# Healthcare-Robotics/assistive-gym

Hardware: AMD Instinct MI355X
Metric: env_steps_per_sec (higher is better)
Workload: dtype f32; 1 GPU; FeedingJaco-v1, 4096 lockstep envs per MI355X, random-policy rollout, 5 simulation steps per env step, 50 PGS sweeps; envs_per_gpu=4096, global_envs=4096, reset_pool=256, reset=pool, parallelism=env-sharded x1, obs_allgather=False

## Files before the change

### __graft_entry__.py

```python
import os
import subprocess
import sys

ROOT = os.path.dirname(os.path.abspath(__file__))
if ROOT not in sys.path:
    sys.path.insert(0, ROOT)


def build():
    from assistive_gym_amd.build import build as build_lib
    build_lib(force=True)
    build_lib(out=os.path.join(ROOT, 'assistive_gym_amd', 'lib', 'variants', 'lvs.so'), extra=('-DAGX_PGS_LV=3',), only=['FEEDING'])
    build_lib(out=os.path.join(ROOT, 'assistive_gym_amd', 'lib', 'variants', 'scan4.so'), extra=('-DAGX_GJK_SCAN_WIDE=0', '-DAGX_GJK_SCAN_ONE=0'), only=['FEEDING'])
    build_lib(out=os.path.join(ROOT, 'assistive_gym_amd', 'lib', 'variants', 'finishgjk.so'), extra=('-DAGX_FINISH_SPILL_GJK',), only=['FEEDING'])
    subprocess.check_call(['make', '-C', os.path.join(ROOT, 'oracle')], stdout=subprocess.DEVNULL)
    if os.path.isdir('/root/reference/assistive_gym/envs/assets'):
        from assistive_gym_amd.model import compiler
        compiler.main()
    import assistive_gym_amd
    from assistive_gym_amd import libagx
    L = libagx.load()
    missing = [e for e in libagx.EXPORTS if not hasattr(L, e)]
    assert not missing, missing


def smoke():
    import numpy as np
    sys.path.insert(0, os.path.join(ROOT, 'tests'))
    from assistive_gym_amd import libagx
    from assistive_gym_amd.blob import ModelBlob
    from assistive_gym_amd.vec_env import build_reset_pool
    from oracle_lib import Oracle
    libagx.check(libagx.load().agx_selftest(0), 'agx_selftest')
    n = 64
    for model in ('feeding_jaco', 'bed_bathing_sawyer'):
        blob = ModelBlob.load(model)
        states = build_reset_pool(blob, n, seed=1001)
        st = libagx.Stepper(blob, n)
        st.set_state(states)
        actions = np.random.RandomState(0).uniform(-1, 1, (n, blob.act_dim)).astype(np.float32)
        obs, rew, done, info = st.step_host(actions)
        o = Oracle(blob)
        worst = 0.0
        for i in range(8):
            o_obs, o_rew, _, o_info = o.step(states[i].copy(), actions[i])
            worst = max(worst, float(np.abs(obs[i] - o_obs).max()), abs(float(rew[i]) - o_rew))
        assert np.isfinite(obs).all() and np.isfinite(rew).all()
        assert worst < 1e-3, (model, worst)
        print('smoke ok: 64 %s envs stepped on the GPU (%s kernels), max |obs, reward| deviation from the oracle %.2e' % (model, st.variant(), worst))
        st.close()


if __name__ == '__main__':
    build()
    if len(sys.argv) > 1 and sys.argv[1] == 'smoke':
        smoke()
```

### assistive_gym_amd/csrc/agx_collide.h

```cpp
#pragma once

namespace agx {

struct Cand { v3 pa, pb, n; float dist, gap; };
constexpr float GJK_FAR_MARGIN = 1e-4f;

AGX_DEV void make_shape(const Ctx& c, int col, v3 shift, gjk_shape& s) {
  s.n = CLI(c, col, AGX_C_NVERT);
  s.v = c.bf + c.o_vert + 3 * CLI(c, col, AGX_C_VOFF);
  v3 p; body_xf(c, CLI(c, col, AGX_C_BODY), s.R, p);
  s.p = p - shift; s.box = false;
  s.c = mul(s.R, mk3(CLF(c, col, AGX_C_AABB_C), CLF(c, col, AGX_C_AABB_C + 1), CLF(c, col, AGX_C_AABB_C + 2))) + s.p;
}
AGX_DEV bool narrowphase(const Ctx& c, int ca, int cb, float limit, Cand& out, bool has) {
  const float* AB = c.lds + L_ARENA;
  gjk_shape sa, sb;
  sa.v = nullptr; sa.n = 0; sa.box = false; sa.c = mk3(0.f, 0.f, 0.f); sb.v = nullptr; sb.n = 0; sb.box = false; sb.c = sa.c;
  v3 shift = mk3(0.f, 0.f, 0.f);
  float ra = 0.f, rb = 0.f;
  bool ok = has;
  if (has) {
    shift = mk3(0.5f * (AB[ABS * ca] + AB[ABS * ca + 3]), 0.5f * (AB[ABS * ca + 1] + AB[ABS * ca + 4]), 0.5f * (AB[ABS * ca + 2] + AB[ABS * ca + 5]));
    make_shape(c, ca, shift, sa); make_shape(c, cb, shift, sb);
    if (CLI(c, cb, AGX_C_BODY) == AGX_BODY_WORLD && sb.n == 8 && (CLI(c, cb, AGX_C_TAG) == AGX_TAG_TABLE || CLI(c, cb, AGX_C_TAG) == AGX_TAG_PLANE)) {
      sb.box = true;
      float lo[3], hi[3];
      for (int k = 0; k < 3; k++) {
        lo[k] = fmaxf(AB[ABS * cb + k], AB[ABS * ca + k] - AGX_BOX_CLIP); hi[k] = fminf(AB[ABS * cb + 3 + k], AB[ABS * ca + 3 + k] + AGX_BOX_CLIP);
        if (hi[k] < lo[k]) ok = false;
      }
      sb.lo = mk3(lo[0], lo[1], lo[2]) - shift; sb.hi = mk3(hi[0], hi[1], hi[2]) - shift; sb.c = 0.5f * (sb.lo + sb.hi);
    }
    ra = CLF(c, ca, AGX_C_RADIUS); rb = CLF(c, cb, AGX_C_RADIUS);
  }
  float d; v3 pa, pb, n;
  const bool pen = gjk_distance(sa, sb, PRM(c, AGX_P_GJK_TOL), (int)PRM(c, AGX_P_GJK_MAXIT), limit + ra + rb + GJK_FAR_MARGIN, ok, d, pa, pb);
  if (!ok) return false;
  if (!pen) {
    if (d - ra - rb >= limit) return false;
    n = (1.0f / d) * (pa - pb);
  } else {
    float depth; gjk_penetration(sa, sb, c.bf + c.o_dirs, c.bi[AGX_H_NDIR], depth, n, pa, pb);
    d = -depth;
  }
  out.pa = pa - ra * n + shift; out.pb = pb + rb * n + shift; out.n = n; out.dist = d - ra - rb;
  return true;
}
AGX_DEV float pair_mu(const Ctx& c, int ca, int cb) {
  float plane_mu = c.lds[L_ST + c.s_env + AGX_E_PLANE_FRICTION];
  float mua = CLI(c, ca, AGX_C_TAG) == AGX_TAG_PLANE ? plane_mu : CLF(c, ca, AGX_C_FRICTION);
  float mub = CLI(c, cb, AGX_C_TAG) == AGX_TAG_PLANE ? plane_mu : CLF(c, cb, AGX_C_FRICTION);
  return mua * mub;
}
AGX_DEV void emit_contact(Ctx& c, int slot, int ca, int cb, const Cand& k) {
  float* o = c.gcon + CON_STRIDE * slot; int* oi = (int*)o;
  oi[C_CA] = ca; oi[C_CB] = cb; oi[C_BA] = CLI(c, ca, AGX_C_BODY); oi[C_BB] = CLI(c, cb, AGX_C_BODY);
  st3(o + C_PA, k.pa); st3(o + C_PB, k.pb); st3(o + C_N, k.n); o[C_DIST] = k.dist; o[C_MU] = pair_mu(c, ca, cb); o[C_LAM] = 0.f;
}
constexpr int CAND_STRIDE = 8;
constexpr int TW_WORDS = 6 * (MAX_DOF + MAX_FREE);
constexpr int WL_FIT = (ARENA_WORDS - ABS * MAX_COLL - TW_WORDS) / (1 + CAND_STRIDE);
constexpr int WL_MAX = WL_FIT < 200 ? WL_FIT : 200;
constexpr int A_WL = ABS * MAX_COLL;
constexpr int WL_KEY_MASK = ~((511 << 9) | (3 << 24));
constexpr int A_CAND = A_WL + WL_MAX;
constexpr int A_TW = A_CAND + WL_MAX * CAND_STRIDE;
static_assert(A_TW + TW_WORDS <= ARENA_WORDS, "collision workspace exceeds the arena");
static_assert(MAX_COLL <= 512, "collider indices are packed in 9 bits");
constexpr bool LIST_BYTES = MAX_COLL <= 256;
constexpr int LIST_TAIL = LIST_BYTES ? 8 : 16;
constexpr int WL_CAP = WL_MAX - LIST_TAIL;
template <bool B> struct ListIndex { typedef unsigned short type; };
template <> struct ListIndex<true> { typedef uint8_t type; };
typedef ListIndex<LIST_BYTES>::type list_t;
static_assert(WL_CAP >= 128, "a flush of at least two full passes");

AGX_DEV void emit_from_cand(Ctx& c, int slot, int idx) {
  const float* L = c.lds; const int pr = c.ldsi[L_ARENA + A_WL + idx]; const float* cd = L + L_ARENA + A_CAND + CAND_STRIDE * idx;
  Cand k; k.gap = cd[0]; k.pa = ld3(cd + 1); k.n = ld3(cd + 4); k.dist = cd[7]; k.pb = k.pa - k.dist * k.n;
  emit_contact(c, slot, pr & 511, (pr >> 9) & 511, k);
}
AGX_DEV bool face_box(const Ctx& c, int cb) {
  return CLI(c, cb, AGX_C_BODY) == AGX_BODY_WORLD && CLI(c, cb, AGX_C_NVERT) == 8 && (CLI(c, cb, AGX_C_TAG) == AGX_TAG_TABLE || CLI(c, cb, AGX_C_TAG) == AGX_TAG_PLANE);
}
AGX_DEV bool face_point(const Ctx& c, int ca, int cb, int e, v3 p0, Cand& out) {
  const float* AB = c.lds + L_ARENA;
  const int n = CLI(c, ca, AGX_C_NVERT);
  const float* V = c.bf + c.o_vert + 3 * CLI(c, ca, AGX_C_VOFF);
  m3 R; v3 p; body_xf(c, CLI(c, ca, AGX_C_BODY), R, p);
  const float x0 = AB[ABS * cb], y0 = AB[ABS * cb + 1], x1 = AB[ABS * cb + 3], y1 = AB[ABS * cb + 4], top = AB[ABS * cb + 5];
  float zmin = 3.0e38f;
  for (int v = 0; v < n; v++) { const v3 w = mul(R, mk3(V[3 * v], V[3 * v + 1], V[3 * v + 2])) + p; if (w.x >= x0 && w.x <= x1 && w.y >= y0 && w.y <= y1 && w.z < zmin) zmin = w.z; }
  float cx[1 + AGX_FACE_EXTRA], cy[1 + AGX_FACE_EXTRA];
  cx[0] = p0.x; cy[0] = p0.y;
#pragma unroll
  for (int q = 1; q <= AGX_FACE_EXTRA; q++) { cx[q] = 0.f; cy[q] = 0.f; }
  v3 pick = mk3(0.f, 0.f, 0.f);
  if (e == 0) {
    bool found = false;
    for (int v = 0; v < n && !found; v++) {
      const v3 w = mul(R, mk3(V[3 * v], V[3 * v + 1], V[3 * v + 2])) + p;
      if (w.x >= x0 && w.x <= x1 && w.y >= y0 && w.y <= y1 && w.z <= zmin + AGX_FACE_BAND) { pick = w; found = true; }
    }
    if (!found) return false;
  }
#pragma unroll
  for (int q = 1; q <= AGX_FACE_EXTRA; q++) {
    if (q > e) break;
    int bi = -1; float bd = AGX_FACE_SPREAD * AGX_FACE_SPREAD; v3 bw = mk3(0.f, 0.f, 0.f);
    for (int v = 0; v < n; v++) {
      const v3 w = mul(R, mk3(V[3 * v], V[3 * v + 1], V[3 * v + 2])) + p;
      if (!(w.x >= x0 && w.x <= x1 && w.y >= y0 && w.y <= y1) || w.z > zmin + AGX_FACE_BAND) continue;
      float dmin = 3.0e38f;
#pragma unroll
      for (int k = 0; k <= AGX_FACE_EXTRA; k++) if (k < q) { const float dx = w.x - cx[k], dy = w.y - cy[k]; dmin = fminf(dmin, dx * dx + dy * dy); }
      if (dmin > bd) { bd = dmin; bi = v; bw = w; }
    }
    if (bi < 0) return false;
    cx[q] = bw.x; cy[q] = bw.y; pick = bw;
  }
  const float ra = CLF(c, ca, AGX_C_RADIUS);
  out.n = mk3(0.f, 0.f, 1.f); out.pa = mk3(pick.x, pick.y, pick.z - ra); out.pb = mk3(pick.x, pick.y, top); out.dist = pick.z - ra - top;
  return true;
}
struct CollideState { int ncon, near_mask, overflow, maxc, nqpt; };
struct GroupRegs { int a0, a1, b0, b1, flags, keep; float alo[3], ahi[3], blo[3], bhi[3]; };
AGX_DEV float body_wmag(const Ctx& c, int code) {
  if (code >= 0 && code < AGX_BODY_ROBOT_BASE) return c.lds[L_WMAG + code];
  if (code >= AGX_BODY_FREE0 && code < AGX_BODY_HUMAN0) return c.lds[L_WMAG + MAX_DOF + (code - AGX_BODY_FREE0)];
  return 0.f;
}
AGX_DEV void body_twist(const Ctx& c, int code, v3& w, v3& v) {
  int slot = -1;
  if (code >= 0 && code < AGX_BODY_ROBOT_BASE) slot = code;
  else if (code >= AGX_BODY_FREE0 && code < AGX_BODY_HUMAN0) slot = MAX_DOF + (code - AGX_BODY_FREE0);
  if (slot < 0) { w = mk3(0.f, 0.f, 0.f); v = w; return; }
  const float* T = c.lds + L_ARENA + A_TW + 6 * slot;
  w = ld3(T); v = ld3(T + 3);
}
AGX_DEV float rel_travel(const Ctx& c, int a, int b) {
  const float* AB = c.lds + L_ARENA;
#ifdef AGX_NO_REL_TRAVEL
  return AB[ABS * a + 6] + AB[ABS * b + 6];
#endif
  v3 wa, va, wb, vb;
  body_twist(c, CLI(c, a, AGX_C_BODY), wa, va); body_twist(c, CLI(c, b, AGX_C_BODY), wb, vb);
  const bool sa = CLI(c, a, AGX_C_NVERT) == 1, sb = CLI(c, b, AGX_C_NVERT) == 1;
  const int e = (!sa && sb) ? b : a;
  const v3 lo = ld3(AB + ABS * e), hi = ld3(AB + ABS * e + 3);
  const v3 ce = 0.5f * (lo + hi), d = hi - lo;
  const v3 dw = wa - wb;
  const v3 u = (va - vb) + cross(dw, ce - ld3(c.lds + L_MISC + M_REF));
  const float rot = (sa || sb) ? 0.f : sqrtf(dot(dw, dw)) * 0.5f * sqrtf(dot(d, d));
  const float t = 1.001f * (sqrtf(dot(u, u)) + rot) * c.dt + 1e-6f;
  return fminf(t, AB[ABS * a + 6] + AB[ABS * b + 6]);
}
AGX_DEV bool sphere_box_apart(const Ctx& c, int x, int y, float reach) {
  const float* AB = c.lds + L_ARENA;
  const v3 cx = mk3(0.5f * (AB[ABS * x] + AB[ABS * x + 3]), 0.5f * (AB[ABS * x + 1] + AB[ABS * x + 4]), 0.5f * (AB[ABS * x + 2] + AB[ABS * x + 5]));
  const v3 hx = mk3(CLF(c, x, AGX_C_AABB_H), CLF(c, x, AGX_C_AABB_H + 1), CLF(c, x, AGX_C_AABB_H + 2));
  const float rx = sqrtf(dot(hx, hx)) + CLF(c, x, AGX_C_RADIUS);
  m3 R; v3 p; body_xf(c, CLI(c, y, AGX_C_BODY), R, p);
  const v3 pl = tmul(R, cx - p) - mk3(CLF(c, y, AGX_C_AABB_C), CLF(c, y, AGX_C_AABB_C + 1), CLF(c, y, AGX_C_AABB_C + 2));
  const float dx = fmaxf(fabsf(pl.x) - CLF(c, y, AGX_C_AABB_H), 0.f), dy = fmaxf(fabsf(pl.y) - CLF(c, y, AGX_C_AABB_H + 1), 0.f),
              dz = fmaxf(fabsf(pl.z) - CLF(c, y, AGX_C_AABB_H + 2), 0.f);
  const float lb = sqrtf(dx * dx + dy * dy + dz * dz) - rx - CLF(c, y, AGX_C_RADIUS);
  return lb > reach;
}

AGX_DEV void collide_flush(Ctx& c, int wn, CollideState& cs, float brk, float slack, const GroupRegs& G) {
  float* L = c.lds; int* WL = c.ldsi + L_ARENA + A_WL; float* CD = L + L_ARENA + A_CAND; const int lane = c.lane;
  const float* AB = L + L_ARENA;
  const int food0 = c.bi[AGX_H_FOOD0];
  if (wn == 0) return;
  wave_sync();
  long long ct0 = c.timing ? wave_clock() : 0;
  if (c.timing) { c.tm[13] += wn; c.tm[14] += (wn + 63) / 64; }
  bool any_manifold_query = false;
  for (int base = 0; base < wn; base += 64) {
    const int i = base + lane; const bool has = i < wn;
    Cand k; k.gap = 3.0e38f; bool near = false; int a = 0, g = 0;
    int b = 0, sub = 0;
    float lim = brk;
    if (has) {
      const int pr = WL[i]; a = pr & 511; b = (pr >> 9) & 511; g = (pr >> 18) & 63; sub = (pr >> 24) & 3;
      if (!(GRI(c, g, AGX_G_FLAGS) & (2 | 64))) lim = fminf(brk, slack + rel_travel(c, a, b) + 1e-5f);
    }
    k.n = mk3(0.f, 0.f, 0.f); k.pa = k.n; k.pb = k.n; k.dist = 0.f;
    bool hit = narrowphase(c, a, b, lim, k, has && sub == 0);
    if (has && sub == 0 && hit && k.n.z > 0.999f && face_box(c, b) && CLI(c, a, AGX_C_NVERT) >= 2) { Cand k0; k0.gap = k.gap; if (face_point(c, a, b, 0, k.pa, k0)) k = k0; }
    if (wave_any(has && sub > 0)) {
      if (has && sub == 0) { float* cd = CD + CAND_STRIDE * i; st3(cd + 1, k.pa); st3(cd + 4, k.n); }
      wave_sync();
      if (has && sub > 0) {
        const float* sd = CD + CAND_STRIDE * (i - sub);
        hit = sd[6] > 0.999f && face_point(c, a, b, sub, ld3(sd + 1), k) && k.dist < brk;
      }
    }
    if (has) {
      if (hit) {
        near = true;
        v3 vr = point_velocity(c, CLI(c, a, AGX_C_BODY), k.pa) - point_velocity(c, CLI(c, b, AGX_C_BODY), k.pb);
        float pg = k.dist + dot(vr, k.n) * c.dt;
        if (pg < ((GRI(c, g, AGX_G_FLAGS) & 64) ? brk : slack)) k.gap = pg;
      }
      float* cd = CD + CAND_STRIDE * i;
      cd[0] = k.gap; st3(cd + 1, k.pa); st3(cd + 4, k.n); cd[7] = k.dist;
    }
    if constexpr (TASK == AGX_TASK_FEEDING) {
      const bool mq = has && near && (GRI(c, g, AGX_G_FLAGS) & 2) && CLI(c, a, AGX_C_TAG) == AGX_TAG_FOOD;
      if (wave_any(mq)) { any_manifold_query = true; for (int f = 0; f < c.nfood; f++) if (wave_any(mq && CLI(c, a, AGX_C_BODY) - AGX_BODY_FREE0 - food0 == f)) cs.near_mask |= 1 << f; }
    }
    if constexpr (TASK != AGX_TASK_FEEDING) {
      const bool qp = has && near && (GRI(c, g, AGX_G_FLAGS) & 2) && CLI(c, a, AGX_C_TAG) == AGX_TAG_TOOL && (TKI(c, AGX_T_PAD_LINK) >> (CLI(c, a, AGX_C_LINK) + 1) & 1) &&
                      CLI(c, b, AGX_C_TAG) == AGX_TAG_HUMAN;
      const uint64_t qm = wave_ballot(qp);
      const int slot = cs.nqpt + wave_rank(qm);
      if (qp && slot < MAX_QPT) { float* o = c.gqpt + QPT_STRIDE * slot; st3(o, k.pb); ((int*)o)[3] = CLI(c, b, AGX_C_LINK); }
      cs.nqpt += popc64(qm);
    }
  }
  (void)any_manifold_query;
  wave_sync();
  if (c.timing) { long long t = wave_clock(); c.tm[11] += t - ct0; ct0 = t; }
  int* SEL = c.ldsi + L_ARENA + A_CAND + CAND_STRIDE * WL_CAP;
  const int ncon0 = cs.ncon;
  int cur = 0;
  while (cur < wn) {
    const int key = WL[cur] & WL_KEY_MASK;
    const int g = (key >> 18) & 63, keep = wave_bcast_i(G.keep, g);
    const int i0 = cur + lane, i1 = cur + 64 + lane;
    const bool s0 = i0 < wn && (WL[i0 < wn ? i0 : 0] & WL_KEY_MASK) == key, s1 = i1 < wn && (WL[i1 < wn ? i1 : 0] & WL_KEY_MASK) == key;
    const uint64_t b0 = wave_ballot(s0), b1 = wave_ballot(s1);
    const int len0 = (~b0) ? ffs64(~b0) : 64;
    const int len = len0 < 64 ? len0 : 64 + ((~b1) ? ffs64(~b1) : 64);
    const bool in0 = lane < len, in1 = 64 + lane < len;
    float g0 = in0 ? CD[CAND_STRIDE * i0] : 3.0e38f, g1 = in1 ? CD[CAND_STRIDE * i1] : 3.0e38f;
    if (keep == 0) {
      for (int pass = 0; pass < 2; pass++) {
        const bool has = (pass ? g1 : g0) < 1.0e38f;
        const uint64_t m = wave_ballot(has);
        int cnt = popc64(m); const int slot = cs.ncon + wave_rank(m);
        if (has && slot < cs.maxc) SEL[slot - ncon0] = pass ? i1 : i0;
        int room = cs.maxc - cs.ncon; if (room < 0) room = 0;
        if (cnt > room) { cs.overflow += cnt - room; cnt = room; }
        cs.ncon += cnt;
      }
    } else {
      for (int q = 0; q < keep; q++) {
        const float mg = wave_min(fminf(g0, g1));
        if (mg > 1.0e38f) break;
        const uint64_t m0 = wave_ballot(g0 == mg);
        int slot1 = 0, win;
        if (m0) win = ffs64(m0); else { win = ffs64(wave_ballot(g1 == mg)); slot1 = 1; }
        if (cs.ncon < cs.maxc) { if (lane == win) SEL[cs.ncon - ncon0] = slot1 ? i1 : i0; cs.ncon++; } else cs.overflow++;
        if (lane == win) { if (slot1) g1 = 3.0e38f; else g0 = 3.0e38f; }
      }
    }
    cur += len;
  }
  wave_sync();
  if (ncon0 + lane < cs.ncon) emit_from_cand(c, ncon0 + lane, SEL[lane]);
  wave_sync();
  if (c.timing) { long long t = wave_clock(); c.tm[12] += t - ct0; }
}

AGX_DEV int collide_sweep(Ctx& c, int g, int aa, int ab, int b0, int b1, int gflags, float mg, int wn, int rep, const GroupRegs& G) {
  const float* AB = c.lds + L_ARENA; int* WL = c.ldsi + L_ARENA + A_WL; const int lane = c.lane;
  const bool same = gflags & 1, no_adjacent = gflags & 4;
  float ulo[2][3], uhi[2][3];
  for (int q = 0; q < 3; q++) { ulo[0][q] = wave_bcast(G.blo[q], g); uhi[0][q] = wave_bcast(G.bhi[q], g); ulo[1][q] = wave_bcast(G.alo[q], g); uhi[1][q] = wave_bcast(G.ahi[q], g); }
  list_t* LIST = (list_t*)(c.ldsi + L_ARENA + A_CAND + CAND_STRIDE * WL_CAP);
  int nlive[2] = {0, 0};
  for (int side = 0; side < 2; side++) {
    const int r0 = side == 0 ? aa : b0, r1 = side == 0 ? ab : b1;
    for (int base = r0; base < r1; base += 64) {
      const int x = base + lane; bool ok = x < r1;
      if (ok) for (int q = 0; q < 3; q++) if (AB[ABS * x + q] > uhi[side][q] + mg || ulo[side][q] > AB[ABS * x + 3 + q] + mg) ok = false;
      const uint64_t m = wave_ballot(ok);
      if (ok) LIST[128 * side + nlive[side] + wave_rank(m)] = (list_t)x;
      nlive[side] += popc64(m);
    }
  }
  const int na_live = nlive[0], nb = nlive[1];
  wave_sync();
  const int npairs = na_live * nb * rep;
  for (int base = 0; base < npairs; base += 64) {
    const int p = base + lane; bool ok = p < npairs;
    const int pq = ok ? p / rep : 0, sub = ok ? p - pq * rep : 0;
    const int ai = pq / nb; const int a = LIST[ai], b = LIST[128 + pq - ai * nb];
    ok = ok && (!same || b > a) && (sub == 0 || (face_box(c, b) && CLI(c, a, AGX_C_NVERT) >= 2));
    if (ok && no_adjacent) {
      const int la = CLI(c, a, AGX_C_BODY), lb = CLI(c, b, AGX_C_BODY);
      if (la == lb) ok = false;
      else if (la >= 0 && la < AGX_BODY_ROBOT_BASE && lb >= 0 && lb < AGX_BODY_ROBOT_BASE && (RBI(c, la, AGX_R_PARENT) == lb || RBI(c, lb, AGX_R_PARENT) == la)) ok = false;
    }
    if (ok) for (int q = 0; q < 3; q++) if (AB[ABS * a + q] > AB[ABS * b + 3 + q] + mg || AB[ABS * b + q] > AB[ABS * a + 3 + q] + mg) ok = false;
    if (ok) { const float reach = mg + rel_travel(c, a, b) + 1e-5f; ok = !sphere_box_apart(c, a, b, reach) && (CLI(c, a, AGX_C_NVERT) == 1 || !sphere_box_apart(c, b, a, reach)); }
    const uint64_t m = wave_ballot(ok);
    const int slot = wn + wave_rank(m);
    if (ok && slot < WL_CAP) WL[slot] = a | (b << 9) | (g << 18) | (sub << 24);
    wn += popc64(m);
  }
  wave_sync();
  return wn;
}

AGX_DEV void collide(Ctx& c) {
  float* L = c.lds; float* AB = L + L_ARENA; const int lane = c.lane;
  const float brk = PRM(c, AGX_P_CONTACT_BREAK), slack = PRM(c, AGX_P_CONTACT_SLACK);
  CollideState cs; cs.ncon = 0; cs.near_mask = 0; cs.overflow = 0; cs.nqpt = 0;
  cs.maxc = (int)PRM(c, AGX_P_MAX_CONTACTS); if (cs.maxc > MAX_CON) cs.maxc = MAX_CON;
  long long ct0 = c.timing ? wave_clock() : 0, ct1;
#define AGX_CTICK(k) if (c.timing) { ct1 = wave_clock(); c.tm[k] += ct1 - ct0; ct0 = ct1; }
  if (lane < MAX_DOF + MAX_FREE) {
    v3 w = mk3(0, 0, 0), v = w;
    if (lane < MAX_DOF) { if (lane < c.ndof) for (int d = lane; d >= 0; d = RBI(c, d, AGX_R_PARENT)) { const float qd = L[L_VEL + d]; w = w + qd * ld3(L + L_S + 6 * d); v = v + qd * ld3(L + L_S + 6 * d + 3); } }
    else if (lane - MAX_DOF < c.nfree) {
      const int fb = lane - MAX_DOF, o = c.ndof + 6 * fb;
      w = ld3(L + L_VEL + o + 3);
      v = ld3(L + L_VEL + o) + cross(w, ld3(L + L_MISC + M_REF) - ld3(L + L_ST + c.s_free + 13 * fb));
    }
    L[L_WMAG + lane] = sqrtf(dot(w, w));
    st3(AB + A_TW + 6 * lane, w); st3(AB + A_TW + 6 * lane + 3, v);
  }
  wave_sync();
  for (int col = lane; col < c.ncoll; col += 64) {
    const int code = CLI(c, col, AGX_C_BODY);
    m3 R; v3 p; body_xf(c, code, R, p);
    v3 cl = mk3(CLF(c, col, AGX_C_AABB_C), CLF(c, col, AGX_C_AABB_C + 1), CLF(c, col, AGX_C_AABB_C + 2));
    v3 hl = mk3(CLF(c, col, AGX_C_AABB_H), CLF(c, col, AGX_C_AABB_H + 1), CLF(c, col, AGX_C_AABB_H + 2));
    v3 cw = mul(R, cl) + p; float r = CLF(c, col, AGX_C_RADIUS);
    v3 vc = point_velocity(c, code, cw);
    const float wmag = body_wmag(c, code);
    const float grow = (sqrtf(dot(vc, vc)) + wmag * (sqrtf(dot(hl, hl)) + r)) * c.dt;
    for (int k = 0; k < 3; k++) {
      float h = fabsf(R.a[3 * k]) * hl.x + fabsf(R.a[3 * k + 1]) * hl.y + fabsf(R.a[3 * k + 2]) * hl.z + r;
      AB[ABS * col + k] = comp(cw, k) - h - grow; AB[ABS * col + 3 + k] = comp(cw, k) + h + grow;
    }
    AB[ABS * col + 6] = grow;
  }
  wave_sync();
  AGX_CTICK(8)
  const int gender = c.ldsi[L_ST + c.s_env + AGX_E_GENDER];
  uint64_t live_groups = 0;
  GroupRegs G; G.a0 = 0; G.a1 = 0; G.b0 = 0; G.b1 = 0; G.flags = 0; G.keep = 0;
  for (int k = 0; k < 3; k++) { G.alo[k] = 0.f; G.ahi[k] = 0.f; G.blo[k] = 0.f; G.bhi[k] = 0.f; }
  {
    const int g = lane; bool live = false;
    if (g < c.ngroup) {
      G.a0 = GRI(c, g, AGX_G_A0); G.a1 = GRI(c, g, AGX_G_A1); G.b0 = GRI(c, g, AGX_G_B0); G.b1 = GRI(c, g, AGX_G_B1);
      if (gender == 1 && GRI(c, g, AGX_G_B0F) >= 0) { G.b0 = GRI(c, g, AGX_G_B0F); G.b1 = GRI(c, g, AGX_G_B1F); }
      G.flags = GRI(c, g, AGX_G_FLAGS); G.keep = GRI(c, g, AGX_G_KEEP);
      const int a0 = G.a0, a1 = G.a1, b0 = G.b0, b1 = G.b1;
      const float mg = (G.flags & (2 | 64)) ? brk : slack;
      const bool wanted = !((G.flags & 8) && gender != 0) && !((G.flags & 16) && gender != 1) &&
                          !((G.flags & 32) && c.nrobot + c.nhdof <= 32 && ((~c.frozen >> c.nrobot) & ((1u << c.nhdof) - 1u)) == 0);
      if (a1 > a0 && b1 > b0 && wanted) {
        float alo[3] = {3.0e38f, 3.0e38f, 3.0e38f}, ahi[3] = {-3.0e38f, -3.0e38f, -3.0e38f}, blo[3] = {3.0e38f, 3.0e38f, 3.0e38f}, bhi[3] = {-3.0e38f, -3.0e38f, -3.0e38f};
        for (int i = a0; i < a1; i++) for (int k = 0; k < 3; k++) { alo[k] = fminf(alo[k], AB[ABS * i + k]); ahi[k] = fmaxf(ahi[k], AB[ABS * i + 3 + k]); }
        for (int i = b0; i < b1; i++) for (int k = 0; k < 3; k++) { blo[k] = fminf(blo[k], AB[ABS * i + k]); bhi[k] = fmaxf(bhi[k], AB[ABS * i + 3 + k]); }
        live = true;
        for (int k = 0; k < 3; k++) if (alo[k] > bhi[k] + mg || blo[k] > ahi[k] + mg) live = false;
        for (int k = 0; k < 3; k++) { G.alo[k] = alo[k]; G.ahi[k] = ahi[k]; G.blo[k] = blo[k]; G.bhi[k] = bhi[k]; }
      }
    }
    live_groups = wave_ballot(live);
  }
  AGX_CTICK(9)
  int wn = 0, g = 0, ab = -1, abatch = 0;
  while (true) {
    while (g < c.ngroup && !(live_groups >> g & 1)) g++;
    if (g >= c.ngroup) {
      if (wn == 0) break;
    } else {
      const int a0 = wave_bcast_i(G.a0, g), a1 = wave_bcast_i(G.a1, g), b0 = wave_bcast_i(G.b0, g), b1 = wave_bcast_i(G.b1, g);
      const int gflags = wave_bcast_i(G.flags, g);
      const float mg = (gflags & (2 | 64)) ? brk : slack;
      const int rep = face_box(c, b0) ? 1 + AGX_FACE_EXTRA : 1;
      const int nb = (b1 - b0) * rep;
      if (ab < 0) { ab = a0; abatch = a1 - a0; }
      const int ae = ab + abatch < a1 ? ab + abatch : a1;
      int wn2 = collide_sweep(c, g, ab, ae, b0, b1, gflags, mg, wn, rep, G);
      AGX_CTICK(10)
      bool fits = wn2 <= WL_CAP;
      if (!fits && wn == 0) {
        const int small = WL_CAP / nb > 0 ? WL_CAP / nb : 1;
        if (abatch > small) { abatch = small; continue; }
        cs.overflow += wn2 - WL_CAP; wn2 = WL_CAP; fits = true;
      }
      if (fits) {
        wn = wn2; ab = ae;
        if (ab >= a1) { g++; ab = -1; }
        if (ab < 0) continue;
      }
    }
    collide_flush(c, wn, cs, brk, slack, G); wn = 0;
    ct0 = c.timing ? wave_clock() : 0;
  }
  c.ncon = cs.ncon; c.near_mask = cs.near_mask; c.overflow = cs.overflow; c.nqpt = cs.nqpt < MAX_QPT ? cs.nqpt : MAX_QPT;
  wave_sync();
#undef AGX_CTICK
}

}
```

Measured before the change: 623,300 env-steps/s.

## Prune narrowphase pairs with conservative lower bounds before evaluating candidates

```diff
diff --git a/__graft_entry__.py b/__graft_entry__.py
--- a/__graft_entry__.py
+++ b/__graft_entry__.py
@@ -13,6 +13,7 @@
     build_lib(out=os.path.join(ROOT, 'assistive_gym_amd', 'lib', 'variants', 'lvs.so'), extra=('-DAGX_PGS_LV=3',), only=['FEEDING'])
     build_lib(out=os.path.join(ROOT, 'assistive_gym_amd', 'lib', 'variants', 'scan4.so'), extra=('-DAGX_GJK_SCAN_WIDE=0', '-DAGX_GJK_SCAN_ONE=0'), only=['FEEDING'])
     build_lib(out=os.path.join(ROOT, 'assistive_gym_amd', 'lib', 'variants', 'finishgjk.so'), extra=('-DAGX_FINISH_SPILL_GJK',), only=['FEEDING'])
+    build_lib(out=os.path.join(ROOT, 'assistive_gym_amd', 'lib', 'variants', 'selectall.so'), extra=('-DAGX_SELECT_ALL_PAIRS',), only=['FEEDING', 'SCRATCH_ITCH'])
     subprocess.check_call(['make', '-C', os.path.join(ROOT, 'oracle')], stdout=subprocess.DEVNULL)
     if os.path.isdir('/root/reference/assistive_gym/envs/assets'):
         from assistive_gym_amd.model import compiler
diff --git a/assistive_gym_amd/csrc/agx_collide.h b/assistive_gym_amd/csrc/agx_collide.h
--- a/assistive_gym_amd/csrc/agx_collide.h
+++ b/assistive_gym_amd/csrc/agx_collide.h
@@ -62,7 +62,8 @@
 constexpr int WL_FIT = (ARENA_WORDS - ABS * MAX_COLL - TW_WORDS) / (1 + CAND_STRIDE);
 constexpr int WL_MAX = WL_FIT < 200 ? WL_FIT : 200;
 constexpr int A_WL = ABS * MAX_COLL;
-constexpr int WL_KEY_MASK = ~((511 << 9) | (3 << 24));
+constexpr int WL_ELIG = 1 << 26, WL_DONE = 1 << 27, WL_TAKE = 1 << 28;
+constexpr int WL_KEY_MASK = ~((511 << 9) | (3 << 24) | WL_ELIG | WL_DONE | WL_TAKE);
 constexpr int A_CAND = A_WL + WL_MAX;
 constexpr int A_TW = A_CAND + WL_MAX * CAND_STRIDE;
 static_assert(A_TW + TW_WORDS <= ARENA_WORDS, "collision workspace exceeds the arena");
@@ -74,6 +75,7 @@
 template <> struct ListIndex<true> { typedef uint8_t type; };
 typedef ListIndex<LIST_BYTES>::type list_t;
 static_assert(WL_CAP >= 128, "a flush of at least two full passes");
+static_assert(WL_CAP <= 256 && WL_CAP <= 4 * LIST_TAIL * CAND_STRIDE, "the pass list holds worklist indices as bytes in the list area");
 
 AGX_DEV void emit_from_cand(Ctx& c, int slot, int idx) {
   const float* L = c.lds; const int pr = c.ldsi[L_ARENA + A_WL + idx]; const float* cd = L + L_ARENA + A_CAND + CAND_STRIDE * idx;
@@ -138,7 +140,7 @@
   const float* T = c.lds + L_ARENA + A_TW + 6 * slot;
   w = ld3(T); v = ld3(T + 3);
 }
-AGX_DEV float rel_travel(const Ctx& c, int a, int b) {
+AGX_DEV float rel_travel(const Ctx& c, int a, int b, v3* travel = nullptr) {
   const float* AB = c.lds + L_ARENA;
 #ifdef AGX_NO_REL_TRAVEL
   return AB[ABS * a + 6] + AB[ABS * b + 6];
@@ -152,10 +154,21 @@
   const v3 dw = wa - wb;
   const v3 u = (va - vb) + cross(dw, ce - ld3(c.lds + L_MISC + M_REF));
   const float rot = (sa || sb) ? 0.f : sqrtf(dot(dw, dw)) * 0.5f * sqrtf(dot(d, d));
+  if (travel) *travel = c.dt * u;
   const float t = 1.001f * (sqrtf(dot(u, u)) + rot) * c.dt + 1e-6f;
   return fminf(t, AB[ABS * a + 6] + AB[ABS * b + 6]);
 }
-AGX_DEV bool sphere_box_apart(const Ctx& c, int x, int y, float reach) {
+#if !defined(AGX_SELECT_ALL_PAIRS) && !defined(AGX_NO_REL_TRAVEL)
+#define AGX_SELECT_BOUNDED
+#endif
+#ifndef AGX_SELECT_S1
+#define AGX_SELECT_S1 8
+#endif
+constexpr float SELECT_EPS = 5.0e-5f;
+#ifndef AGX_TRACE_BOUND
+#define AGX_TRACE_BOUND(a, b, elig, lb, pg)
+#endif
+AGX_DEV bool sphere_box_apart(const Ctx& c, int x, int y, float reach, bool want_bound = false, v3 w = v3(), float* bound = nullptr) {
   const float* AB = c.lds + L_ARENA;
   const v3 cx = mk3(0.5f * (AB[ABS * x] + AB[ABS * x + 3]), 0.5f * (AB[ABS * x + 1] + AB[ABS * x + 4]), 0.5f * (AB[ABS * x + 2] + AB[ABS * x + 5]));
   const v3 hx = mk3(CLF(c, x, AGX_C_AABB_H), CLF(c, x, AGX_C_AABB_H + 1), CLF(c, x, AGX_C_AABB_H + 2));
@@ -164,9 +177,101 @@
   const v3 pl = tmul(R, cx - p) - mk3(CLF(c, y, AGX_C_AABB_C), CLF(c, y, AGX_C_AABB_C + 1), CLF(c, y, AGX_C_AABB_C + 2));
   const float dx = fmaxf(fabsf(pl.x) - CLF(c, y, AGX_C_AABB_H), 0.f), dy = fmaxf(fabsf(pl.y) - CLF(c, y, AGX_C_AABB_H + 1), 0.f),
               dz = fmaxf(fabsf(pl.z) - CLF(c, y, AGX_C_AABB_H + 2), 0.f);
-  const float lb = sqrtf(dx * dx + dy * dy + dz * dz) - rx - CLF(c, y, AGX_C_RADIUS);
+  const float s0 = sqrtf(dx * dx + dy * dy + dz * dz);
+  const float lb = s0 - rx - CLF(c, y, AGX_C_RADIUS);
+  if (want_bound) {
+    const v3 p1 = pl + tmul(R, w);
+    const float ex = fmaxf(fabsf(p1.x) - CLF(c, y, AGX_C_AABB_H), 0.f), ey = fmaxf(fabsf(p1.y) - CLF(c, y, AGX_C_AABB_H + 1), 0.f), ez = fmaxf(fabsf(p1.z) - CLF(c, y, AGX_C_AABB_H + 2), 0.f);
+    const float ww = dot(w, w);
+    *bound = s0 > sqrtf(ww) + SELECT_EPS ? sqrtf(ex * ex + ey * ey + ez * ez) - ww / (2.0f * s0) - (rx + CLF(c, y, AGX_C_RADIUS)) - SELECT_EPS : -3.0e38f;
+  }
   return lb > reach;
 }
+
+AGX_DEV int segment_len(const int* WL, int cur, int wn, int lane) {
+  const int key = WL[cur] & WL_KEY_MASK;
+  const int i0 = cur + lane, i1 = cur + 64 + lane;
+  const bool s0 = i0 < wn && (WL[i0 < wn ? i0 : 0] & WL_KEY_MASK) == key, s1 = i1 < wn && (WL[i1 < wn ? i1 : 0] & WL_KEY_MASK) == key;
+  const uint64_t b0 = wave_ballot(s0), b1 = wave_ballot(s1);
+  const int len0 = (~b0) ? ffs64(~b0) : 64;
+  return len0 < 64 ? len0 : 64 + ((~b1) ? ffs64(~b1) : 64);
+}
+#ifndef AGX_SELECT_ALL_PAIRS
+AGX_DEV int select_stage(Ctx& c, int wn, int stage, float slack, const GroupRegs& G) {
+  int* WL = c.ldsi + L_ARENA + A_WL; float* CD = c.lds + L_ARENA + A_CAND; const int lane = c.lane;
+  uint8_t* PL = (uint8_t*)(c.ldsi + L_ARENA + A_CAND + CAND_STRIDE * WL_CAP);
+  int first = wn, last = -1;
+  for (int base = 0; base < wn; base += 64) {
+    const int i = base + lane;
+    const bool pend = i < wn && (WL[i < wn ? i : 0] & (WL_ELIG | WL_DONE)) == WL_ELIG;
+    const uint64_t m = wave_ballot(pend);
+    if (m) { if (last < 0) first = base + ffs64(m); last = base + 63 - clz64(m); }
+  }
+  while (last >= 0) {
+    const int j = first - 1 - lane;
+    const uint64_t m = wave_ballot(j >= 0 && ((WL[j >= 0 ? j : 0] ^ WL[first]) & WL_KEY_MASK) == 0);
+    const int back = (~m) ? ffs64(~m) : 64;
+    first -= back;
+    if (back < 64) break;
+  }
+  for (int cur = first; cur <= last;) {
+    const int len = segment_len(WL, cur, wn, lane);
+    const int keep = wave_bcast_i(G.keep, (WL[cur] >> 18) & 63);
+    const int i0 = cur + lane, i1 = cur + 64 + lane; const bool in0 = lane < len, in1 = 64 + lane < len;
+    const int w0 = in0 ? WL[i0] : 0, w1 = in1 ? WL[i1] : 0;
+    const bool e0 = (w0 & (WL_ELIG | WL_DONE)) == WL_ELIG, e1 = (w1 & (WL_ELIG | WL_DONE)) == WL_ELIG;
+    if (wave_any(e0 || e1)) {
+      const float l0 = e0 ? CD[CAND_STRIDE * i0] : 3.0e38f, l1 = e1 ? CD[CAND_STRIDE * i1] : 3.0e38f;
+      bool t0, t1;
+#ifdef AGX_SELECT_EVAL_ALL
+      const bool all = true;
+#else
+      const bool all = len >= 128;
+#endif
+      if (all) { t0 = e0; t1 = e1; }
+      else if (stage == 0) {
+        t0 = e0 && l0 < -1.0e38f; t1 = e1 && l1 < -1.0e38f;
+        float c0 = (e0 && !t0 && l0 < slack) ? l0 : 3.0e38f, c1 = (e1 && !t1 && l1 < slack) ? l1 : 3.0e38f;
+        for (int q = popc64(wave_ballot(t0)) + popc64(wave_ballot(t1)); q < AGX_SELECT_S1; q++) {
+          const float mb = wave_min(fminf(c0, c1));
+          if (mb > 1.0e38f) break;
+          const uint64_t m0 = wave_ballot(c0 == mb);
+          if (m0) { if (lane == ffs64(m0)) { t0 = true; c0 = 3.0e38f; } }
+          else if (lane == ffs64(wave_ballot(c1 == mb))) { t1 = true; c1 = 3.0e38f; }
+        }
+      } else {
+        float g0 = (in0 && (w0 & WL_DONE)) ? CD[CAND_STRIDE * i0] : 3.0e38f, g1 = (in1 && (w1 & WL_DONE)) ? CD[CAND_STRIDE * i1] : 3.0e38f;
+        float tau = slack;
+        for (int q = 0; q < keep; q++) {
+          const float mg = wave_min(fminf(g0, g1));
+          if (mg > 1.0e38f) break;
+          if (q == keep - 1) tau = mg;
+          const uint64_t m0 = wave_ballot(g0 == mg);
+          if (m0) { if (lane == ffs64(m0)) g0 = 3.0e38f; }
+          else if (lane == ffs64(wave_ballot(g1 == mg))) g1 = 3.0e38f;
+        }
+        t0 = e0 && l0 < slack && l0 <= tau; t1 = e1 && l1 < slack && l1 <= tau;
+        if (e0 && !t0) CD[CAND_STRIDE * i0] = 3.0e38f;
+        if (e1 && !t1) CD[CAND_STRIDE * i1] = 3.0e38f;
+      }
+      if (t0) WL[i0] = w0 | WL_TAKE;
+      if (t1) WL[i1] = w1 | WL_TAKE;
+    }
+    cur += len;
+  }
+  wave_sync();
+  int n = 0;
+  for (int base = 0; base < wn; base += 64) {
+    const int i = base + lane; const int w = i < wn ? WL[i] : WL_DONE;
+    const bool take = !(w & WL_DONE) && ((w & WL_TAKE) || (stage == 1 && !(w & WL_ELIG)));
+    const uint64_t m = wave_ballot(take);
+    if (take) { PL[n + wave_rank(m)] = (uint8_t)i; WL[i] = (w | WL_DONE) & ~WL_TAKE; }
+    n += popc64(m);
+  }
+  wave_sync();
+  return n;
+}
+#endif
 
 AGX_DEV void collide_flush(Ctx& c, int wn, CollideState& cs, float brk, float slack, const GroupRegs& G) {
   float* L = c.lds; int* WL = c.ldsi + L_ARENA + A_WL; float* CD = L + L_ARENA + A_CAND; const int lane = c.lane;
@@ -175,10 +280,23 @@
   if (wn == 0) return;
   wave_sync();
   long long ct0 = c.timing ? wave_clock() : 0;
-  if (c.timing) { c.tm[13] += wn; c.tm[14] += (wn + 63) / 64; }
   bool any_manifold_query = false;
-  for (int base = 0; base < wn; base += 64) {
-    const int i = base + lane; const bool has = i < wn;
+#ifdef AGX_SELECT_ALL_PAIRS
+  for (int stage = 0; stage < 1; stage++) {
+  const int np = wn;
+#else
+  const uint8_t* PL = (const uint8_t*)(c.ldsi + L_ARENA + A_CAND + CAND_STRIDE * WL_CAP);
+  for (int stage = 0; stage < 2; stage++) {
+  const int np = select_stage(c, wn, stage, slack, G);
+#endif
+  if (c.timing) { c.tm[13] += np; c.tm[14] += (np + 63) / 64; }
+  for (int base = 0; base < np; base += 64) {
+    const bool has = base + lane < np;
+#ifdef AGX_SELECT_ALL_PAIRS
+    const int i = base + lane;
+#else
+    const int i = has ? PL[base + lane] : 0;
+#endif
     Cand k; k.gap = 3.0e38f; bool near = false; int a = 0, g = 0;
     int b = 0, sub = 0;
     float lim = brk;
@@ -203,7 +321,8 @@
         v3 vr = point_velocity(c, CLI(c, a, AGX_C_BODY), k.pa) - point_velocity(c, CLI(c, b, AGX_C_BODY), k.pb);
         float pg = k.dist + dot(vr, k.n) * c.dt;
         if (pg < ((GRI(c, g, AGX_G_FLAGS) & 64) ? brk : slack)) k.gap = pg;
-      }
+        AGX_TRACE_BOUND(a, b, WL[i] & WL_ELIG, CD[CAND_STRIDE * i], pg)
+      } else { AGX_TRACE_BOUND(a, b, WL[i] & WL_ELIG, CD[CAND_STRIDE * i], 3.0e38f) }
       float* cd = CD + CAND_STRIDE * i;
       cd[0] = k.gap; st3(cd + 1, k.pa); st3(cd + 4, k.n); cd[7] = k.dist;
     }
@@ -220,6 +339,7 @@
       cs.nqpt += popc64(qm);
     }
   }
+  }
   (void)any_manifold_query;
   wave_sync();
   if (c.timing) { long long t = wave_clock(); c.tm[11] += t - ct0; ct0 = t; }
@@ -227,13 +347,9 @@
   const int ncon0 = cs.ncon;
   int cur = 0;
   while (cur < wn) {
-    const int key = WL[cur] & WL_KEY_MASK;
-    const int g = (key >> 18) & 63, keep = wave_bcast_i(G.keep, g);
+    const int g = (WL[cur] >> 18) & 63, keep = wave_bcast_i(G.keep, g);
     const int i0 = cur + lane, i1 = cur + 64 + lane;
-    const bool s0 = i0 < wn && (WL[i0 < wn ? i0 : 0] & WL_KEY_MASK) == key, s1 = i1 < wn && (WL[i1 < wn ? i1 : 0] & WL_KEY_MASK) == key;
-    const uint64_t b0 = wave_ballot(s0), b1 = wave_ballot(s1);
-    const int len0 = (~b0) ? ffs64(~b0) : 64;
-    const int len = len0 < 64 ? len0 : 64 + ((~b1) ? ffs64(~b1) : 64);
+    const int len = segment_len(WL, cur, wn, lane);
     const bool in0 = lane < len, in1 = 64 + lane < len;
     float g0 = in0 ? CD[CAND_STRIDE * i0] : 3.0e38f, g1 = in1 ? CD[CAND_STRIDE * i1] : 3.0e38f;
     if (keep == 0) {
@@ -268,6 +384,10 @@
 AGX_DEV int collide_sweep(Ctx& c, int g, int aa, int ab, int b0, int b1, int gflags, float mg, int wn, int rep, const GroupRegs& G) {
   const float* AB = c.lds + L_ARENA; int* WL = c.ldsi + L_ARENA + A_WL; const int lane = c.lane;
   const bool same = gflags & 1, no_adjacent = gflags & 4;
+#ifdef AGX_SELECT_BOUNDED
+  const bool bounded = wave_bcast_i(G.keep, g) > 0 && !(gflags & (2 | 64));
+  float* CD = c.lds + L_ARENA + A_CAND;
+#endif
   float ulo[2][3], uhi[2][3];
   for (int q = 0; q < 3; q++) { ulo[0][q] = wave_bcast(G.blo[q], g); uhi[0][q] = wave_bcast(G.bhi[q], g); ulo[1][q] = wave_bcast(G.alo[q], g); uhi[1][q] = wave_bcast(G.ahi[q], g); }
   list_t* LIST = (list_t*)(c.ldsi + L_ARENA + A_CAND + CAND_STRIDE * WL_CAP);
@@ -296,10 +416,22 @@
       else if (la >= 0 && la < AGX_BODY_ROBOT_BASE && lb >= 0 && lb < AGX_BODY_ROBOT_BASE && (RBI(c, la, AGX_R_PARENT) == lb || RBI(c, lb, AGX_R_PARENT) == la)) ok = false;
     }
     if (ok) for (int q = 0; q < 3; q++) if (AB[ABS * a + q] > AB[ABS * b + 3 + q] + mg || AB[ABS * b + q] > AB[ABS * a + 3 + q] + mg) ok = false;
+#ifdef AGX_SELECT_BOUNDED
+    const bool elig = ok && bounded && sub == 0 && CLI(c, a, AGX_C_NVERT) == 1 && !face_box(c, b);
+    float bound = -3.0e38f;
+    if (ok) { v3 w; const float reach = mg + rel_travel(c, a, b, &w) + 1e-5f; ok = !sphere_box_apart(c, a, b, reach, elig, w, &bound) && (CLI(c, a, AGX_C_NVERT) == 1 || !sphere_box_apart(c, b, a, reach)); }
+#else
     if (ok) { const float reach = mg + rel_travel(c, a, b) + 1e-5f; ok = !sphere_box_apart(c, a, b, reach) && (CLI(c, a, AGX_C_NVERT) == 1 || !sphere_box_apart(c, b, a, reach)); }
+#endif
     const uint64_t m = wave_ballot(ok);
     const int slot = wn + wave_rank(m);
-    if (ok && slot < WL_CAP) WL[slot] = a | (b << 9) | (g << 18) | (sub << 24);
+    if (ok && slot < WL_CAP) {
+      int word = a | (b << 9) | (g << 18) | (sub << 24);
+#ifdef AGX_SELECT_BOUNDED
+      if (elig) { CD[CAND_STRIDE * slot] = bound; word |= WL_ELIG; }
+#endif
+      WL[slot] = word;
+    }
     wn += popc64(m);
   }
   wave_sync();
```

Result: slower. 614,200 env-steps/s (-1.5%).

## Compute face contact points before GJK and skip narrowphase when provably resting on box face

Applied to the files above, without the earlier changes.

```diff
diff --git a/__graft_entry__.py b/__graft_entry__.py
--- a/__graft_entry__.py
+++ b/__graft_entry__.py
@@ -13,6 +13,7 @@
     build_lib(out=os.path.join(ROOT, 'assistive_gym_amd', 'lib', 'variants', 'lvs.so'), extra=('-DAGX_PGS_LV=3',), only=['FEEDING'])
     build_lib(out=os.path.join(ROOT, 'assistive_gym_amd', 'lib', 'variants', 'scan4.so'), extra=('-DAGX_GJK_SCAN_WIDE=0', '-DAGX_GJK_SCAN_ONE=0'), only=['FEEDING'])
     build_lib(out=os.path.join(ROOT, 'assistive_gym_amd', 'lib', 'variants', 'finishgjk.so'), extra=('-DAGX_FINISH_SPILL_GJK',), only=['FEEDING'])
+    build_lib(out=os.path.join(ROOT, 'assistive_gym_amd', 'lib', 'variants', 'faceplain.so'), extra=('-DAGX_FACE_PLAIN',), only=['FEEDING', 'FEEDING_M'])
     subprocess.check_call(['make', '-C', os.path.join(ROOT, 'oracle')], stdout=subprocess.DEVNULL)
     if os.path.isdir('/root/reference/assistive_gym/envs/assets'):
         from assistive_gym_amd.model import compiler
diff --git a/assistive_gym_amd/csrc/agx_collide.h b/assistive_gym_amd/csrc/agx_collide.h
--- a/assistive_gym_amd/csrc/agx_collide.h
+++ b/assistive_gym_amd/csrc/agx_collide.h
@@ -123,6 +123,73 @@
   out.n = mk3(0.f, 0.f, 1.f); out.pa = mk3(pick.x, pick.y, pick.z - ra); out.pb = mk3(pick.x, pick.y, top); out.dist = pick.z - ra - top;
   return true;
 }
+#ifdef AGX_FACE_PLAIN
+#undef AGX_FACE
+#define AGX_FACE 0
+#endif
+#ifndef AGX_FACE
+#define AGX_FACE 2
+#endif
+#if AGX_FACE < 0 || AGX_FACE > 2
+#error "AGX_FACE: 0, 1 or 2"
+#endif
+constexpr float FACE_PROOF_GUARD = 1e-4f, FACE_PROOF_GUARD_LIM = 1e-5f;
+
+#if AGX_FACE
+AGX_DEV bool face_point_wide(const Ctx& c, int ca, int cb, int e, v3 p0, float& zmin, Cand& out) {
+  const float* AB = c.lds + L_ARENA;
+  const int n = CLI(c, ca, AGX_C_NVERT), last = n - 1;
+  const float* V = c.bf + c.o_vert + 3 * CLI(c, ca, AGX_C_VOFF);
+  m3 R; v3 p; body_xf(c, CLI(c, ca, AGX_C_BODY), R, p);
+  const float x0 = AB[ABS * cb], y0 = AB[ABS * cb + 1], x1 = AB[ABS * cb + 3], y1 = AB[ABS * cb + 4], top = AB[ABS * cb + 5];
+#define FACE_LDV(j, kk) const int i##j = (kk) < last ? (kk) : last; const float vx##j = V[3 * i##j], vy##j = V[3 * i##j + 1], vz##j = V[3 * i##j + 2];
+#define FACE_LD8(k) FACE_LDV(0, k) FACE_LDV(1, k + 1) FACE_LDV(2, k + 2) FACE_LDV(3, k + 3) FACE_LDV(4, k + 4) FACE_LDV(5, k + 5) FACE_LDV(6, k + 6) FACE_LDV(7, k + 7)
+#define FACE_W(j) const v3 w = mul(R, mk3(vx##j, vy##j, vz##j)) + p; const bool in = w.x >= x0 && w.x <= x1 && w.y >= y0 && w.y <= y1;
+#define FACE_ALL8(F) F(0) F(1) F(2) F(3) F(4) F(5) F(6) F(7)
+#define FACE_FRESH(i) (mul(R, mk3(V[3 * (i)], V[3 * (i) + 1], V[3 * (i) + 2])) + p)
+  float cx[1 + AGX_FACE_EXTRA], cy[1 + AGX_FACE_EXTRA];
+  cx[0] = p0.x; cy[0] = p0.y;
+#pragma unroll
+  for (int q = 1; q <= AGX_FACE_EXTRA; q++) { cx[q] = 0.f; cy[q] = 0.f; }
+  v3 pick = mk3(0.f, 0.f, 0.f);
+  if (e == 0) {
+    int iz = -1; float zm = 3.0e38f;
+#define FACE_ZMIN(j) { FACE_W(j) const bool t = in && w.z < zm; zm = t ? w.z : zm; iz = t ? i##j : iz; }
+    for (int k = 0; k < n; k += 8) { FACE_LD8(k) FACE_ALL8(FACE_ZMIN) }
+#undef FACE_ZMIN
+    zmin = 3.0e38f;
+    if (iz < 0) return false;
+    zmin = FACE_FRESH(iz).z;
+    int first = -1;
+#define FACE_BAND(j) { FACE_W(j) const bool t = first < 0 && in && w.z <= zmin + AGX_FACE_BAND; first = t ? i##j : first; }
+    for (int k = 0; k < n && first < 0; k += 8) { FACE_LD8(k) FACE_ALL8(FACE_BAND) }
+#undef FACE_BAND
+    if (first < 0) return false;
+    pick = FACE_FRESH(first);
+  }
+#pragma unroll
+  for (int q = 1; q <= AGX_FACE_EXTRA; q++) {
+    if (q > e) break;
+    int bi = -1; float bd = AGX_FACE_SPREAD * AGX_FACE_SPREAD;
+#define FACE_FAR(j) { FACE_W(j) float dmin = 3.0e38f; \
+      _Pragma("unroll") for (int kk = 0; kk <= AGX_FACE_EXTRA; kk++) if (kk < q) { const float dx = w.x - cx[kk], dy = w.y - cy[kk]; dmin = fminf(dmin, dx * dx + dy * dy); } \
+      const bool t = in && !(w.z > zmin + AGX_FACE_BAND) && dmin > bd; bd = t ? dmin : bd; bi = t ? i##j : bi; }
+    for (int k = 0; k < n; k += 8) { FACE_LD8(k) FACE_ALL8(FACE_FAR) }
+#undef FACE_FAR
+    if (bi < 0) return false;
+    const v3 bw = FACE_FRESH(bi);
+    cx[q] = bw.x; cy[q] = bw.y; pick = bw;
+  }
+#undef FACE_LDV
+#undef FACE_LD8
+#undef FACE_W
+#undef FACE_ALL8
+#undef FACE_FRESH
+  const float ra = CLF(c, ca, AGX_C_RADIUS);
+  out.n = mk3(0.f, 0.f, 1.f); out.pa = mk3(pick.x, pick.y, pick.z - ra); out.pb = mk3(pick.x, pick.y, top); out.dist = pick.z - ra - top;
+  return true;
+}
+#endif
 struct CollideState { int ncon, near_mask, overflow, maxc, nqpt; };
 struct GroupRegs { int a0, a1, b0, b1, flags, keep; float alo[3], ahi[3], blo[3], bhi[3]; };
 AGX_DEV float body_wmag(const Ctx& c, int code) {
@@ -187,14 +254,49 @@
       if (!(GRI(c, g, AGX_G_FLAGS) & (2 | 64))) lim = fminf(brk, slack + rel_travel(c, a, b) + 1e-5f);
     }
     k.n = mk3(0.f, 0.f, 0.f); k.pa = k.n; k.pb = k.n; k.dist = 0.f;
+#if AGX_FACE
+    bool proven = false;
+    if (has && sub == 0) {
+      float* cd = CD + CAND_STRIDE * i; float state = 0.f;
+      if (face_box(c, b) && CLI(c, a, AGX_C_NVERT) >= 2) {
+        Cand k0; k0.pa = k.pa; k0.dist = 0.f; float zmin;
+        const bool first = face_point_wide(c, a, b, 0, k.pa, zmin, k0);
+        st3(cd + 1, k0.pa); cd[7] = k0.dist;
+#pragma unroll
+        for (int q = 1; q <= AGX_FACE_EXTRA; q++) if (i + q < wn) CD[CAND_STRIDE * (i + q)] = zmin;
+        state = first ? 1.f : 0.f;
+#if AGX_FACE >= 2
+        const float* Aa = AB + ABS * a; const float* Bb = AB + ABS * b; const float top = Bb[5], dcore = zmin - top;
+        proven = first && Aa[0] >= Bb[0] + FACE_PROOF_GUARD && Aa[3] <= Bb[3] - FACE_PROOF_GUARD && Aa[1] >= Bb[1] + FACE_PROOF_GUARD && Aa[4] <= Bb[4] - FACE_PROOF_GUARD &&
+                 Aa[0] <= Aa[3] && Aa[1] <= Aa[4] && Aa[2] - AGX_BOX_CLIP <= top && Aa[5] + AGX_BOX_CLIP >= top && Bb[2] <= top &&
+                 dcore > FACE_PROOF_GUARD && dcore - CLF(c, a, AGX_C_RADIUS) - CLF(c, b, AGX_C_RADIUS) < lim - FACE_PROOF_GUARD_LIM;
+        if (proven) state = 2.f;
+#endif
+      }
+      cd[0] = state;
+    }
+    bool hit = narrowphase(c, a, b, lim, k, has && sub == 0 && !proven);
+    if (has && sub == 0) {
+      const float* cd = CD + CAND_STRIDE * i; const float state = cd[0];
+      if (state == 2.f || (state == 1.f && hit && k.n.z > 0.999f)) {
+        hit = true; k.n = mk3(0.f, 0.f, 1.f); k.pa = ld3(cd + 1); k.pb = mk3(k.pa.x, k.pa.y, AB[ABS * b + 5]); k.dist = cd[7];
+      }
+    }
+#else
     bool hit = narrowphase(c, a, b, lim, k, has && sub == 0);
     if (has && sub == 0 && hit && k.n.z > 0.999f && face_box(c, b) && CLI(c, a, AGX_C_NVERT) >= 2) { Cand k0; k0.gap = k.gap; if (face_point(c, a, b, 0, k.pa, k0)) k = k0; }
+#endif
     if (wave_any(has && sub > 0)) {
       if (has && sub == 0) { float* cd = CD + CAND_STRIDE * i; st3(cd + 1, k.pa); st3(cd + 4, k.n); }
       wave_sync();
       if (has && sub > 0) {
         const float* sd = CD + CAND_STRIDE * (i - sub);
+#if AGX_FACE
+        float zmin = CD[CAND_STRIDE * i];
+        hit = sd[6] > 0.999f && face_point_wide(c, a, b, sub, ld3(sd + 1), zmin, k) && k.dist < brk;
+#else
         hit = sd[6] > 0.999f && face_point(c, a, b, sub, ld3(sd + 1), k) && k.dist < brk;
+#endif
       }
     }
     if (has) {
```

Result: faster. 624,500 env-steps/s before, 660,400 env-steps/s after (median of 6 runs) (+5.7%).
